# cvlab-stonybrook/s-volsdf

Hardware: AMD Instinct MI355X
Metric: rendered rays/sec (1024-ray batch, 128 samples) (higher is better)
Workload: dtype f32 (every product, forward and backward, as three fp16 MFMA products of two-piece fp16 operands with f32 accumulate; activation blocks hold both pieces: float32 accuracy class); 1 GPU; configs[1]: VolOpt.train_step (forward + MVS prior lookup + loss + backward + clip/guard/Adam), train mode, fast=1: 1024 rays/GPU x 128 coarse + 98 composited samples + 2048 eikonal points, 8x256 SDF MLP + 4x256 radiance MLP; mode=train, mlp_precision=fp16x2, launch=eager launches, rays_per_gpu=1024, rays_total=1024

## Files before the change

### include/svolsdf_hip.h

```cpp
#ifndef SVOLSDF_HIP_H
#define SVOLSDF_HIP_H

#include <stddef.h>
#include <stdint.h>

#ifdef __cplusplus
extern "C" {
#endif


#define SVS_EINVAL (-1)
#define SVS_ESHAPE (-2)
#define SVS_ENOCONV (-3)
#define SVS_EOVERFLOW (-4)

#define SVS_HOST

#define SVS_ABI_VERSION 101
int svs_version(void);
const char* svs_last_error_string(void);

int svs_set_deterministic(int on);
int svs_get_deterministic(void);

// ... 55 lines not shown
int svs_bg_points(const float* cam, int cam_stride, const float* dirs, int n_rays, int n_bg, const float* jitter,
                  float radius, float* z_bg, float* pts, float* depth_real, void* hip_stream);
int svs_bg_sdf_eval(const float* pts, int n_points, const float* stream, int precision, float* out0, float* feat_tiles,
                    float* hbuf, float* ghat7, float* pebuf, void* hip_stream);
size_t svs_bg_rbuf_bytes(int n_points);
int svs_bg_rgb_eval(int n_points, const float* view_dirs, int view_S, const float* feat_tiles, const float* stream,
                    int precision, float* rgb, float* rbuf, void* hip_stream);
int svs_bg_rgb_bwd(int n_points, const float* d_rgb, const float* rgb, const float* rbuf, const float* stream, int precision,
                   float* zbuf, float* feat_bar, float* absmax, void* hip_stream);
int svs_bg_sdf_bwd(int n_points, const float* d_out0, const float* feat_bar, const float* hbuf, const float* ghat7,
                   const float* stream, int precision, float* abuf, float* sbar_out, float* absmax, void* hip_stream);
int svs_composite_bg(int n_rays, int n_samples, int n_bg, const float* z, const float* z_max, const float* sdf,
                     const float* rgb, const float* normals, const float* depth_scale, const float* beta_param,
                     float beta_min, const float* z_bg, const float* bg_out0, const float* bg_rgb, const float* bg_depth,
                     float* weights, float* bg_trans, float* bg_weights, float* rgb_values, float* depth_values,
                     float* depth_values_all, float* depth_vals, float* normal_map, void* hip_stream);
int svs_composite_bg_bwd(int n_rays, int n_samples, int n_bg, const float* z, const float* z_max, const float* sdf,
                         const float* rgb, const float* depth_scale, const float* beta_param, float beta_min,
                         const float* z_bg, const float* bg_out0, const float* bg_rgb, const float* d_rgb_values,
                         const float* d_weights, const float* d_depth_values, const float* d_depth_all,
                         const float* bg_depth, float* d_sdf, float* d_rgb,
                         float* d_bg_out0, float* d_bg_rgb, float* d_beta_ray, float* d_beta_param, void* hip_stream);

typedef struct svs_wgrad_job {
  const float *a0, *b0; long long sa0, sb0;
  const float *a1, *b1; long long sa1, sb1;
  const float* b_extra; long long s_extra;
  int n_points, ldw;
  float *dW, *db;
  const float* absmax;
  const float *rec0, *rec1;
} svs_wgrad_job;
int svs_wgrad_multi(const svs_wgrad_job* jobs, int n_jobs, int precision, void* hip_stream);
int svs_wgrad(const float* a0, const float* b0, long long sa0, long long sb0, const float* a1, const float* b1,
              long long sa1, long long sb1, const float* b_extra, long long s_extra, int n_points, int precision,
              const float* absmax, const float* rec0, const float* rec1, float* dW, int ldw, float* db, void* hip_stream);

size_t svs_block_bytes(int n_points, int blocks_per_tile);
size_t svs_rgb_zbuf_bytes(int n_points);
size_t svs_sdf_ubuf_bytes(int n_points);
size_t svs_sdf_gbuf_bytes(int n_points);
int svs_rgb_bwd(int n_points, const float* d_rgb, const float* rgb, const float* rbuf, const float* stream, int precision,
                float* zbuf, float* feat_bar, float* d_normals, float* absmax, void* hip_stream);
int svs_sdf_bwd_a(const float* points, int n_points, const float* cam, int cam_stride, const float* dirs, const float* z,
                  int S, int n_rays, const float* d_grad, const unsigned char* clamp_mask, const float* hbuf,
                  const float* gbuf, const float* stream, int precision, float* ubuf, float* a2buf, float* pebuf,
                  float* absmax, void* hip_stream);
int svs_sdf_bwd_b(int n_points, const float* d_sdf, const unsigned char* clamp_mask, const float* feat_bar,
                  int n_feat_points, const float* hbuf, const float* gbuf, const float* a2buf, const float* ubuf,
                  const float* stream, int precision, float* abuf, float* sbar_out, float* absmax, void* hip_stream);
int svs_lin8_row0_grad(const float* hbuf, const float* ubuf, const float* sbar, int n_points, int precision, float* out257,
                       void* hip_stream);
int svs_unpack_wgrad(const float* dWk, const float* dbk, int ldw, int map, int rows, int cols, int row_off,
                     const float* weight_v, const float* weight_g, const float* row0, float* grad_v, float* grad_g,
                     float* grad_b, void* hip_stream);
typedef struct svs_unpack_job {
  const float *dWk, *dbk;
  int ldw, map, rows, cols, row_off;
  const float *weight_v, *weight_g, *row0;
  float *grad_v, *grad_g, *grad_b;
} svs_unpack_job;
int svs_unpack_wgrad_multi(const svs_unpack_job* jobs, int n_jobs, void* hip_stream);

size_t svs_adam_workspace_bytes(void);
int svs_clip_guard_adam(float* params, float* grads, float* exp_avg, float* exp_avg_sq, long long n, int step,
                        int* step_counter, double max_norm, double lr, double beta1, double beta2, double eps,
// ... 282 lines not shown
```

### s-volsdf_amd/csrc/svs_wgrad.hip

```cpp
#include "svs_common.h"
#include "svs_mlp_layout.h"
#include "svs_ticket.h"
#include "svs_wgrad_maps.h"
#include <cstdlib>
#include <type_traits>

namespace svs {
namespace wgrad {

struct Pair {
  const float* a;
  const float* b;
  size_t stride_a, stride_b;
};

struct Args {
  Pair p[2];
  int n_pairs;
  int n_tiles;
  int n_valid_points;
  const float* b_extra;
  size_t stride_extra;
  float* dW;
  int ldw;
// ... 138 lines not shown
  if constexpr (N > 0) {
    static_for<N - 1>(f);
    f(std::integral_constant<int, N - 1>{});
  }
}
__device__ __forceinline__ f16x8 frag_of(const Frag& v) { return __builtin_bit_cast(f16x8, v); }
__device__ __forceinline__ void lds_read128(f32x4& v, unsigned a) { asm volatile("ds_read_b128 %0, %1" : "=v"(v) : "v"(a)); }
__device__ __forceinline__ void lds_read32(float& v, unsigned a) { asm volatile("ds_read_b32 %0, %1" : "=v"(v) : "v"(a)); }
__device__ __forceinline__ void lds_wait() {
  asm volatile("s_waitcnt lgkmcnt(0)" ::: "memory");
  __builtin_amdgcn_sched_barrier(0);
}
__device__ __forceinline__ unsigned lds_addr(const void* p) {
  return (unsigned)(unsigned long long)SVS_LDS(const void, p);
}

__device__ __forceinline__ void scale_from_absmax(const float* absmax, float& s, float& inv_s) {
  s = 1.0f; inv_s = 1.0f;
  if (!absmax) return;
  int e = (int)((__float_as_uint(*absmax) >> 23) & 0xff);
  e = e < 16 ? 16 : (e > 250 ? 250 : e);
  s = __uint_as_float((unsigned)(268 - e) << 23);
  inv_s = __uint_as_float((unsigned)(e - 14) << 23);
}

struct Job {
  Pair p[2];
  const float* rec[2];
  int n_pairs;
  int n_tiles;
  int n_valid_points;
  int b_tiles;
  int col0;
  float* dW;
  int ldw;
  float* db;
  const float* absmax;
  int wg_begin, wg_count;
  det::Ticket ticket;
};
constexpr int kMaxJobs = 20;
struct MultiArgs { Job job[kMaxJobs]; int n_jobs; int touch; int reverse; };
static_assert(sizeof(MultiArgs) <= 4096, "kernel arguments");

constexpr int kThreadsW = 512;
constexpr int kRT = 2, kCT = 16;
static_assert(maps::plane_reads_ok(kPlane), "transposed reads of the operand planes: bank conflict");
static_assert(maps::narrow_reads_ok(kExtraPiece), "transposed reads of the narrow B image: bank conflict");
static_assert(kPlane % 256 == 0 && kNarrowImg % 256 == 0 && kExtraPiece % 256 == 0 && Ring<true>::kSlotAll % 256 == 0 &&
              Ring<false>::kSlotAll % 256 == 0, "every region the reads are offset by starts on a 256-byte bank row");

typedef const __attribute__((address_space(1))) void* gvoid;

template <bool GP>
__global__ __launch_bounds__(kThreadsW, 1) void wgrad_h2_multi_kernel(MultiArgs ma) {
  typedef Ring<GP> R;
  constexpr int kSlot = R::kSlot, kSlotAll = R::kSlotAll, kRing = R::kRing, kAhead = R::kAhead, kB = R::kB;
  extern __shared__ __attribute__((aligned(16))) unsigned char smem_h2[];
  int jj = 0;
  for (int q = 1; q < ma.n_jobs; ++q) if ((int)blockIdx.x >= ma.job[q].wg_begin) jj = q;
  const Job& a = ma.job[jj];
  const int wg = (int)blockIdx.x - a.wg_begin, nwg = a.wg_count;
  const int tid = threadIdx.x, lane = tid & 63;
  const int wave = __builtin_amdgcn_readfirstlane(tid >> 6);
  const bool narrow = a.b_tiles == 1;
  float s_grad, inv_s;
  scale_from_absmax(a.absmax, s_grad, inv_s);

  f32x4 acc[kRT][kCT];
#pragma unroll
  for (int o = 0; o < kRT; ++o)
#pragma unroll
    for (int i = 0; i < kCT; ++i) acc[o][i] = (f32x4)(0.0f);
  float bsum[kRT];
#pragma unroll
  for (int o = 0; o < kRT; ++o) bsum[o] = 0.0f;

  unsigned char* ring = smem_h2;

  const int rg = lane >> 4;
  const int rd_even = maps::plane_base(0, lane), rd_odd = maps::plane_base(1, lane);
  const int a_off = 1024 * kRT * wave;
  const int rx = maps::narrow_base(lane);
  const int wp = lane & 31, whf = lane >> 5;
  const int wxoff = maps::narrow_at(8 * (wave & 3) + 4 * whf, wp);
  const int n_ct = narrow ? 2 : kCT;

  const bool two_pairs = a.n_pairs == 2;
  const int my_tiles = a.n_tiles > wg ? (a.n_tiles - 1 - wg) / nwg + 1 : 0;
  const int n_items = two_pairs ? 2 * my_tiles : my_tiles;
  const int n_valid = a.n_valid_points;
  const bool has_db = a.db != nullptr;
  const bool rev = ma.reverse != 0;
  const float* const pa0 = a.p[0].a; const float* const pb0 = a.p[0].b;
  const float* const pa1 = a.p[1].a; const float* const pb1 = a.p[1].b;
  const size_t sa0 = a.p[0].stride_a, sb0 = a.p[0].stride_b, sa1 = a.p[1].stride_a, sb1 = a.p[1].stride_b;
  const float* const rec0 = a.rec[0]; const float* const rec1 = a.rec[1];
  const bool has_scale = a.absmax != nullptr;
  auto tile_of = [&](int item) {
    const int k = two_pairs ? item >> 1 : item;
    return rev ? wg + (my_tiles - 1 - k) * nwg : wg + k * nwg;
  };

  auto issue = [&](int item) {
    const int t = tile_of(item), pi = two_pairs ? item & 1 : 0;
    const float* pa = (pi ? pa1 : pa0) + (size_t)t * (pi ? sa1 : sa0);
    const float* pb = (pi ? pb1 : pb0) + (size_t)t * (pi ? sb1 : sb0);
    unsigned char* slot = ring + (item % kRing) * kSlotAll;
#pragma unroll
    for (int j = 0; j < 2 * R::kPlanes; ++j) {
      const int piece = wave + 8 * j;
      __builtin_amdgcn_global_load_lds((gvoid)(reinterpret_cast<const f32x4*>(pa) + piece * 64 + lane),
                                       SVS_LDS(void, slot + piece * 1024), 16, 0, 0);
      if (!narrow)
        __builtin_amdgcn_global_load_lds((gvoid)(reinterpret_cast<const f32x4*>(pb) + piece * 64 + lane),
                                         SVS_LDS(void, slot + kB + piece * 1024), 16, 0, 0);
    }
    if (narrow)
      __builtin_amdgcn_global_load_lds((gvoid)(reinterpret_cast<const f32x4*>(pb) + (wave & 3) * 64 + lane),
                                       SVS_LDS(void, slot + kB + (wave & 3) * 1024), 16, 0, 0);
    if (has_scale)
      __builtin_amdgcn_global_load_lds((gvoid)((pi ? rec1 : rec0) + (size_t)t * 64 + lane),
                                       SVS_LDS(void, slot + kSlot + wave * 256), 4, 0, 0);
  };
  unsigned sink = 0;
  auto touch = [&](int item) {
    const int t = tile_of(item), pi = two_pairs ? item & 1 : 0;
    const Pair& p = a.p[pi];
    constexpr int kLines = R::kPlanes * (kPlane / 128);
    const int nb = narrow ? 32 : kLines;
    const float* q = tid < kLines ? p.a + (size_t)t * p.stride_a + tid * 32
                                  : p.b + (size_t)t * p.stride_b + (tid - kLines) * 32;
    if (tid < kLines + nb) asm volatile("global_load_dword %0, %1, off" : "+v"(sink) : "v"(q) : "memory");
  };
  const int ops = (narrow ? 2 * R::kPlanes + 1 : 4 * R::kPlanes) + (has_scale ? 1 : 0);

  auto stage_factors = [&](int item) {
    unsigned char* slot = ring + (item % kRing) * kSlotAll;
    const int t = tile_of(item);
    const int live = n_valid - t * 32;
    float f = 1.0f;
    if (has_scale) {
      float rec;
      lds_read32(rec, lds_addr(slot + kSlot + wave * 256 + 4 * wp));
      lds_wait();
      const unsigned eb = (__float_as_uint(rec) >> 23) & 0xff;
      if (eb >= 20 && eb <= 240) f = __builtin_fminf(s_grad * __uint_as_float((254u << 23) - __float_as_uint(rec)), 32768.0f);
// ... 57 lines not shown
    const unsigned ftab = la + kSlot + kRecBytes + wave * 64;
    const unsigned a_even = la + a_off + rd_even, a_odd = la + a_off + rd_odd;
    const unsigned b_even = lb + rd_even, b_odd = lb + rd_odd;
    const unsigned n_rd = lb + kNarrowImg + rx;
    const bool want_bias = has_db && p0;
    const bool two = narrow;
    Frag fa[kRT], fam[kRT];
    f32x4 fraw;
    static_for<kRT>([&](auto oc) {
      constexpr int o = decltype(oc)::value;
      tr_issue<1024 * o>(fa[o], o & 1 ? a_odd : a_even);
      if (GP) tr_issue<kPlane + 1024 * o>(fam[o], o & 1 ? a_odd : a_even);
    });
    lds_read128(fraw, ftab + 16 * rg);
    issue_next();
    lds_wait();
    f16x8 ah[kRT], am[kRT];
#pragma unroll
    for (int o = 0; o < kRT; ++o) {
      ah[o] = frag_of(fa[o]) * __builtin_bit_cast(f16x8, fraw);
      am[o] = GP ? frag_of(fam[o]) * __builtin_bit_cast(f16x8, fraw) : ah[o];
      if (want_bias) {
#pragma unroll
        for (int j = 0; j < 4; ++j) {
          const f16x2 h2v = {ah[o][2 * j], ah[o][2 * j + 1]};
          bsum[o] = __builtin_amdgcn_fdot2(h2v, one2, bsum[o], false);
          if (GP) {
            const f16x2 m2v = {am[o][2 * j], am[o][2 * j + 1]};
            bsum[o] = __builtin_amdgcn_fdot2(m2v, one2, bsum[o], false);
          }
        }
      }
    }
    static_for<kCT>([&](auto ic) {
      constexpr int i = decltype(ic)::value;
      if (i < n_ct) {
        Frag fh, fm;
        if (!narrow) {
          tr_issue<1024 * i>(fh, i & 1 ? b_odd : b_even);
          if (GP) tr_issue<kPlane + 1024 * i>(fm, i & 1 ? b_odd : b_even);
        } else if constexpr (i < 2) {
          tr_issue<1024 * i>(fh, n_rd);
          tr_issue<kExtraPiece + 1024 * i>(fm, n_rd);
        }
        lds_wait();
        const f16x8 bh = frag_of(fh), bm = frag_of(fm);
        if (two || GP) {
#pragma unroll
          for (int o = 0; o < kRT; ++o) acc[o][i] = __builtin_amdgcn_mfma_f32_16x16x32_f16(ah[o], bm, acc[o][i], 0, 0, 0);
        }
        if (GP) {
#pragma unroll
          for (int o = 0; o < kRT; ++o) acc[o][i] = __builtin_amdgcn_mfma_f32_16x16x32_f16(am[o], bh, acc[o][i], 0, 0, 0);
        }
#pragma unroll
        for (int o = 0; o < kRT; ++o) acc[o][i] = __builtin_amdgcn_mfma_f32_16x16x32_f16(ah[o], bh, acc[o][i], 0, 0, 0);
      }
    });
  }
  asm volatile("s_waitcnt vmcnt(0)" :: "v"(sink) : "memory");
  const int fcol = lane & 15;
  det::wait_turn(a.ticket, wg);
  static_for<kCT>([&](auto ic) {
    constexpr int i = decltype(ic)::value;
    const int c = a.col0 + 16 * i + fcol;
    if (i < n_ct && c < a.ldw) {
#pragma unroll
      for (int o = 0; o < kRT; ++o)
#pragma unroll
        for (int r = 0; r < 4; ++r)
          atomicAdd(&a.dW[(size_t)(16 * (kRT * wave + o) + 4 * rg + r) * a.ldw + c], acc[o][i][r] * inv_s);
    }
  });
  if (a.db) {
#pragma unroll
    for (int o = 0; o < kRT; ++o) {
      float sum = bsum[o];
      sum += __shfl_xor(sum, 16);
      sum += __shfl_xor(sum, 32);
      if (lane < 16) atomicAdd(&a.db[16 * (kRT * wave + o) + lane], sum * inv_s);
    }
  }
  det::pass_turn(a.ticket, wg);
}

}

}
}

using namespace svs;
using namespace svs::wgrad;
namespace h2 = svs::wgrad::h2;

extern "C" {

int svs_wgrad_multi(const svs_wgrad_job* jobs, int n_jobs, int precision, void* hip_stream) {
  if (!jobs || n_jobs < 1) { set_error("svs_wgrad_multi: no jobs"); return SVS_EINVAL; }
  int n_expanded = 0;
  for (int j = 0; j < n_jobs; ++j) n_expanded += jobs[j].b_extra ? 2 : 1;
  if (n_expanded > h2::kMaxJobs) { set_error("svs_wgrad_multi: at most %d jobs (b_extra counts twice)", h2::kMaxJobs); return SVS_EINVAL; }
  for (int j = 0; j < n_jobs; ++j) {
    const svs_wgrad_job& q = jobs[j];
    if (!q.a0 || !q.b0 || !q.dW || q.n_points <= 0 || q.ldw < 256 || q.ldw > 288 || (q.b_extra && q.ldw < 288) || (q.a1 && !q.b1)) {
      set_error("svs_wgrad_multi: bad argument in job %d", j); return SVS_EINVAL;
    }
    if (mlp::is_h2(precision) && q.absmax && (!q.rec0 || (q.a1 && !q.rec1))) {
      set_error("svs_wgrad_multi: job %d has absmax but no scale records", j); return SVS_EINVAL;
    }
  }
  hipStream_t s = (hipStream_t)hip_stream;
  if (mlp::is_h2(precision)) {
    const bool gp = precision == mlp::kFmtF16x2;
    h2::MultiArgs ma;
    int n = 0;
    long long work[h2::kMaxJobs], total = 0;
    for (int j = 0; j < n_jobs; ++j) {
      const svs_wgrad_job& q = jobs[j];
      h2::Job& J = ma.job[n];
      J.p[0] = Pair{q.a0, q.b0, (size_t)q.sa0, (size_t)q.sb0};
      J.rec[0] = q.rec0; J.rec[1] = q.rec1;
      J.n_pairs = 1;
      if (q.a1) { J.p[1] = Pair{q.a1, q.b1, (size_t)q.sa1, (size_t)q.sb1}; J.n_pairs = 2; }
      else { J.p[1] = J.p[0]; J.rec[1] = J.rec[0]; }
      J.n_tiles = (q.n_points + 31) / 32; J.n_valid_points = q.n_points;
      J.b_tiles = 8; J.col0 = 0; J.dW = q.dW; J.ldw = q.ldw; J.db = q.db; J.absmax = q.absmax;
      work[n] = (long long)J.n_tiles * J.n_pairs * 10;
      total += work[n++];
      if (q.b_extra) {
        h2::Job& X = ma.job[n];
        X = J;
        X.p[0].b = q.b_extra; X.p[0].stride_b = (size_t)q.s_extra; X.n_pairs = 1;
        X.b_tiles = 1; X.col0 = 256; X.db = nullptr;
        work[n] = (long long)X.n_tiles * 6;
        total += work[n++];
      }
    }
    ma.n_jobs = n;
    static const int touch_env = [] { const char* e = getenv("SVS_WGRAD_TOUCH"); return e ? atoi(e) : 0; }();
    ma.touch = touch_env;
    static const int reverse_env = [] { const char* e = getenv("SVS_WGRAD_REVERSE"); return e ? atoi(e) : 0; }();
    ma.reverse = reverse_env;
    (void)total;
    const int n_wg_total = 256;
    int count[h2::kMaxJobs];
    int used = 0;
    for (int j = 0; j < n; ++j) { count[j] = 1; ++used; }
    while (used < n_wg_total) {
      int best = -1;
      double load = 0.0;
      for (int j = 0; j < n; ++j) {
        if (count[j] >= ma.job[j].n_tiles) continue;
        const double l = (double)work[j] / count[j];
        if (l > load) { load = l; best = j; }
      }
      if (best < 0) break;
      ++count[best]; ++used;
    }
    int begin = 0;
    for (int j = 0; j < n; ++j) {
      ma.job[j].wg_begin = begin; ma.job[j].wg_count = count[j];
      begin += count[j];
      ma.job[j].ticket = det::Ticket{nullptr, 0u, 0u};
    }
    if (deterministic()) {
      int owner[h2::kMaxJobs], n_owner = 0;
      for (int j = 0; j < n; ++j) {
// ... 20 lines not shown
    return check_launch("svs_wgrad_multi");
  }
  if (precision != mlp::kFmtF32) { set_error("svs_wgrad_multi: unknown precision %d", precision); return SVS_EINVAL; }
  for (int j = 0; j < n_jobs; ++j) {
    const svs_wgrad_job& q = jobs[j];
    Args a;
    a.p[0] = Pair{q.a0, q.b0, (size_t)q.sa0, (size_t)q.sb0};
    a.n_pairs = 1;
    if (q.a1) { a.p[1] = Pair{q.a1, q.b1, (size_t)q.sa1, (size_t)q.sb1}; a.n_pairs = 2; }
    a.n_tiles = (q.n_points + 31) / 32;
    a.n_valid_points = q.n_points;
    a.b_extra = q.b_extra; a.stride_extra = (size_t)q.s_extra;
    a.dW = q.dW; a.ldw = q.ldw; a.db = q.db;
    const int grid = a.n_tiles < 256 ? a.n_tiles : 256;
    a.ticket = det::Ticket{det::take_slots(1), 0u, (unsigned)grid};
    if (q.b_extra) {
      constexpr int lds = 2 * 32 * (260 + 292) * 4;
      static hipError_t e9 = hipFuncSetAttribute(reinterpret_cast<const void*>(wgrad_kernel<9>),
                                                 hipFuncAttributeMaxDynamicSharedMemorySize, lds);
      if (e9 != hipSuccess) { set_error("svs_wgrad_multi: hipFuncSetAttribute: %s", hipGetErrorString(e9)); return (int)e9; }
      wgrad_kernel<9><<<grid, 256, lds, s>>>(a);
    } else {
      constexpr int lds = 2 * 32 * (260 + 260) * 4;
      static hipError_t e8 = hipFuncSetAttribute(reinterpret_cast<const void*>(wgrad_kernel<8>),
                                                 hipFuncAttributeMaxDynamicSharedMemorySize, lds);
      if (e8 != hipSuccess) { set_error("svs_wgrad_multi: hipFuncSetAttribute: %s", hipGetErrorString(e8)); return (int)e8; }
      wgrad_kernel<8><<<grid, 256, lds, s>>>(a);
    }
    if (int rc = check_launch("svs_wgrad_multi")) return rc;
  }
  return SVS_OK;
}

int svs_wgrad(const float* a0, const float* b0, long long sa0, long long sb0, const float* a1, const float* b1,
              long long sa1, long long sb1, const float* b_extra, long long s_extra, int n_points, int precision,
              const float* absmax, const float* rec0, const float* rec1, float* dW, int ldw, float* db, void* hip_stream) {
  svs_wgrad_job q{a0, b0, sa0, sb0, a1, b1, sa1, sb1, b_extra, s_extra, n_points, ldw, dW, db, absmax, rec0, rec1};
  return svs_wgrad_multi(&q, 1, precision, hip_stream);
}

}
```

### s-volsdf_amd/svs_hip/lib.py

```python
import ctypes
import os
import re
from ctypes import POINTER, c_char_p, c_double, c_float, c_int, c_longlong, c_size_t, c_void_p

_HERE = os.path.dirname(os.path.abspath(__file__))
LIB_PATH = os.environ.get("SVS_LIB_PATH") or os.path.join(os.path.dirname(_HERE), "lib", "libsvolsdf_hip.so")
HEADER_PATH = os.path.join(os.path.dirname(os.path.dirname(_HERE)), "include", "svolsdf_hip.h")

_lib = None


class SvsError(RuntimeError):
    pass


_SCALARS = {"int": c_int, "float": c_float, "double": c_double, "size_t": c_size_t, "long long": c_longlong}
_POINTEES = set(_SCALARS) | {"void", "char", "unsigned char", "uint8_t", "short", "unsigned int", "unsigned long long"}
_TOKENS = re.compile(r"\w+|\*").findall
_NOT_A_DECLARATOR = re.compile(r"[^\w\s*]").search


def _ctype(base, stars, host, pointees):
    if stars == 0 and not host:
        return _SCALARS.get(base)
# ... 55 lines not shown
                raise SvsError(f"{HEADER_PATH}: enum: cannot parse `{item}`")
            constants[e.group(1)] = int(e.group(2))
        return " "
    text = re.sub(r"\benum\s*\{([^}]*)\}\s*;", enum, text)

    def struct(m):
        if m.group(1) != m.group(3):
            raise SvsError(f"{HEADER_PATH}: typedef struct {m.group(1)} is named {m.group(3)}")
        structs[m.group(1)] = _struct_fields(m.group(1), m.group(2))
        return " "
    text = re.sub(r"\btypedef\s+struct\s+(\w+)\s*\{([^}]*)\}\s*(\w+)\s*;", struct, text)

    pointees = _POINTEES | set(structs)
    for decl in filter(None, (d.strip() for d in text.split(";"))):
        m = re.fullmatch(r"([\w\s*]+?)\b(\w+)\s*\(([^()]*)\)", decl)
        if not m:
            raise SvsError(f"{HEADER_PATH}: cannot parse declaration `{' '.join(decl.split())[:80]}`")
        name, params = m.group(2), m.group(3).strip()
        _, restype = _declarator(m.group(1) + " " + name, pointees, f"{name}, return type")
        args = [] if params == "void" else [_declarator(p, pointees, name)[1] for p in params.split(",")]
        signatures[name] = (restype, args)
    return constants, structs, signatures


def _structure(cls_name, fields, c_name):
    return type(cls_name, (ctypes.Structure,), {"_fields_": fields, "__doc__": f"{c_name} of include/svolsdf_hip.h"})


try:
    with open(HEADER_PATH) as _f:
        _CONSTANTS, _STRUCTS, SIGNATURES = parse_header(_f.read())
    WGradJob = _structure("WGradJob", _STRUCTS["svs_wgrad_job"], "svs_wgrad_job")
    UnpackJob = _structure("UnpackJob", _STRUCTS["svs_unpack_job"], "svs_unpack_job")
    ABI_VERSION = _CONSTANTS["SVS_ABI_VERSION"]
    EINVAL, ESHAPE, ENOCONV, EOVERFLOW = (_CONSTANTS["SVS_E" + n] for n in ("INVAL", "SHAPE", "NOCONV", "OVERFLOW"))
    MMA_F32, MMA_F16X2, MMA_F16X2_HALF = (_CONSTANTS["SVS_MMA_" + n] for n in ("F32", "F16X2", "F16X2_HALF"))
    PAINT_BEST, PAINT_ONE_SIDED = (_CONSTANTS["SVS_PAINT_" + n] for n in ("BEST", "ONE_SIDED"))
except (OSError, KeyError) as _e:
    raise SvsError(f"{HEADER_PATH}: the binding is derived from this header and cannot do without it: {_e!r}") from _e


def load():
    global _lib
    if _lib is not None:
        return _lib
    import torch
    if not os.path.exists(LIB_PATH):
        raise SvsError(f"{LIB_PATH} not found: run `python s-volsdf_amd/build.py` (there is no CPU fallback)")
    lib = ctypes.CDLL(LIB_PATH)
    for name, (res, args) in SIGNATURES.items():
        fn = getattr(lib, name)
        fn.restype = res
        fn.argtypes = args
    have = lib.svs_version()
    if have != ABI_VERSION:
        raise SvsError(f"{LIB_PATH} has ABI version {have}, the header this binding reads declares {ABI_VERSION}: "
                       "rebuild with `python s-volsdf_amd/build.py --force`")
    if os.environ.get("SVS_DETERMINISTIC") == "1":
        lib.svs_set_deterministic(1)
    _lib = lib
    return lib


def deterministic():
    return bool(load().svs_get_deterministic())

# ... 6 lines not shown
```

### s-volsdf_amd/svs_hip/profiling.py

```python
import torch

from . import lib as _lib


class LaunchTimer:

    def __init__(self, names):
        self.names = list(names)
        self.events = {n: [] for n in self.names}
        self._orig = {}
        self.meta = {n: [] for n in self.names}

    def __enter__(self):
        L = _lib.load()
        for n in self.names:
            fn = getattr(L, n)
            self._orig[n] = fn
            setattr(L, n, self._wrap(n, fn))
        return self

    def _wrap(self, name, fn):
        def call(*args):
            e0, e1 = torch.cuda.Event(enable_timing=True), torch.cuda.Event(enable_timing=True)
            e0.record()
            rc = fn(*args)
            e1.record()
            self.events[name].append((e0, e1))
            self.meta[name].append(args)
            return rc
        return call

    def __exit__(self, *exc):
        L = _lib.load()
        for n, fn in self._orig.items():
            setattr(L, n, fn)
        return False

    def times_ms(self, name):
        return [a.elapsed_time(b) for a, b in self.events[name]]
```

### s-volsdf_amd/svs_hip/train.py

```python
import ctypes
import os

import torch

from . import lib as _lib
from .ops import _f32, _ptr, _ptr_array, _stream, default_precision, is_h2, F16X2, F16X2_HALF

KBLOCK = 128 * 64
KREC = 64


def block_stride(n_points):
    return ((n_points + 127) // 128) * 4 * KBLOCK
LDW = 288


def n_tiles_padded(n_points):
    return ((n_points + 127) // 128) * 4


def record_off(n_points, n_blocks, block):
    T = n_tiles_padded(n_points)
    return n_blocks * T * KBLOCK + block * T * KREC


def _off(t, n_floats):
    return t.data_ptr() + 4 * n_floats


class TrainStreams:
    def __init__(self, device, precision=None):
        L = _lib.load()
        self.precision = default_precision() if precision is None else int(precision)
        self.sdf = torch.empty(L.svs_stream_bytes(2) // 4, device=device)
        self.rgb = torch.empty(L.svs_stream_bytes(4) // 4, device=device)
        self.ws = torch.empty(L.svs_pack_workspace_bytes() // 4, device=device)

    def pack(self, sdf_params, rgb_params):
        L = _lib.load()
        sv, sg, sb = [[_f32(t) for t in x] if x is not None else None for x in sdf_params]
        rv, rg, rb = [[_f32(t) for t in x] if x is not None else None for x in rgb_params]
        self._keep = (sv, sg, sb, rv, rg, rb)
        st = _stream()
        _lib.check(L.svs_pack_stream(2, self.precision, _ptr_array(sv), _ptr_array(sg) if sg else None, _ptr_array(sb), _ptr(self.ws),
                                     _ptr(self.sdf), st), "svs_pack_stream(sdf train)")
        _lib.check(L.svs_pack_stream(4, self.precision, _ptr_array(rv), _ptr_array(rg) if rg else None, _ptr_array(rb), _ptr(self.ws),
                                     _ptr(self.rgb), st), "svs_pack_stream(rgb bwd)")


class WGradAccum:

    def __init__(self, device, slots=14):
        n = [slots * 256 * LDW, slots * 256, 260, 4]
        self.flat = torch.zeros(sum(n), device=device)
        parts = torch.split(self.flat, n)
        self.dWk = parts[0].view(slots, 256, LDW)
        self.dbk = parts[1].view(slots, 256)
        self.row0 = parts[2][:257]
        self.absmax = parts[3]

    def zero(self):
        self.flat.zero_()

    def bases(self):
        return self.dWk.data_ptr(), self.dbk.data_ptr(), self.absmax.data_ptr()


class _JobCache(dict):

    def memo(self, key, build):
        hit = self.get(key)
        if hit is None:
            if len(self) >= 64:
                self.clear()
            hit = self[key] = build()
        return hit


def _job_array(jobs):
    arr = (_lib.WGradJob * len(jobs))(*[_lib.WGradJob(*j) for j in jobs])
    return ctypes.cast(arr, ctypes.c_void_p), len(jobs), arr


def _f(addr, n_floats):
    return addr + 4 * n_floats


def wgrad_job(acc, slot, n_pts, amax, scaled, a0, sa0, b0, sb0, a1=None, sa1=0, b1=None, sb1=0, extra=None, sx=0,
              rec0=None, rec1=None):
    dWk, dbk, absmax = acc
    return (a0, b0, sa0, sb0, a1, b1, sa1, sb1, extra, sx, n_pts, LDW, _f(dWk, slot * 256 * LDW), _f(dbk, slot * 256),
            _f(absmax, amax) if scaled else None, rec0 if scaled else None, rec1 if scaled else None)


def rgb_wgrad_table(n_main, h2, acc, zbuf, feat, rbuf):
    LSm = block_stride(n_main)
    zrec = lambda l: _f(zbuf, record_off(n_main, 5, l))
    jobs = [wgrad_job(acc, 9, n_main, 1, h2, zbuf, KBLOCK, feat, KBLOCK, extra=_f(rbuf, 4 * LSm), sx=1024, rec0=zrec(0))]
    for l in range(1, 5):
        jobs.append(wgrad_job(acc, 9 + l, n_main, 1, h2, _f(zbuf, l * LSm), KBLOCK, _f(rbuf, (l - 1) * LSm), KBLOCK,
                              rec0=zrec(l)))
    return jobs


def sdf_wgrad_table(n_total, n_main, h2, acc, abuf, ubuf, pebuf, hbuf, gbuf, feat_bar):
    LS = block_stride(n_total)
    arec = lambda l: _f(abuf, record_off(n_total, 8, l))
    second = lambda l: dict(a1=_f(gbuf, l * LS), sa1=KBLOCK, b1=_f(ubuf, l * LS), sb1=KBLOCK,
                            rec1=_f(ubuf, record_off(n_total, 9, l)))
    jobs = [wgrad_job(acc, 0, n_total, 0, h2, abuf, KBLOCK, pebuf, KBLOCK, rec0=arec(0), **second(0))]
    for l in range(1, 8):
        jobs.append(wgrad_job(acc, l, n_total, 0, h2, _f(abuf, l * LS), KBLOCK, _f(hbuf, (l - 1) * LS), KBLOCK, rec0=arec(l),
                              **second(l)))
    jobs.append(wgrad_job(acc, 8, n_main, 2, h2, feat_bar, KBLOCK, _f(hbuf, 7 * LS), KBLOCK,
                          rec0=_f(feat_bar, record_off(n_main, 1, 0))))
    return jobs


BGRBUF = KBLOCK + 1024


def bg_wgrad_table(P, acc, abuf, zbuf, feat_bar, hbuf, pebuf, rbuf, feat):
    LS, Z2, T = block_stride(P), 2 * KBLOCK, n_tiles_padded(P)
    job = lambda slot, amax, *a, **k: wgrad_job(acc, slot, P, amax, True, *a, **k)
    arec = lambda l: _f(abuf, record_off(P, 8, l))
    jobs = [job(0, 0, abuf, KBLOCK, pebuf, KBLOCK, rec0=arec(0))]
    for l in range(1, 8):
        jobs.append(job(l, 0, _f(abuf, l * LS), KBLOCK, _f(hbuf, (l - 1) * LS), KBLOCK, rec0=arec(l)))
    jobs.append(job(8, 2, feat_bar, KBLOCK, _f(hbuf, 7 * LS), KBLOCK, rec0=_f(feat_bar, record_off(P, 1, 0))))
    zrec = lambda b: _f(zbuf, 2 * T * KBLOCK + b * T * KREC)
    jobs.append(job(9, 1, zbuf, Z2, feat, KBLOCK, rec0=zrec(0), extra=_f(rbuf, KBLOCK), sx=BGRBUF))
    jobs.append(job(10, 1, _f(zbuf, KBLOCK), Z2, rbuf, BGRBUF, rec0=zrec(1)))
    return jobs


def unpack_table(dWk, dbk, row0, layers, maps):
    jobs = []
    for net, l, slot, rows, cols, v, g, gv, gg, gb in layers:
        mp = maps[0] if (net == 0 and l == 4) else (maps[1] if (net == 1 and l == 0) else 0)
        last = net == 0 and l == 8
        jobs.append((_f(dWk, slot * 256 * LDW), _f(dbk, slot * 256), LDW, mp, rows, cols, 1 if last else 0, v, g,
                     row0 if last else None, gv, gg, gb))
    return jobs


def _unpack(accum, nets, maps, out, which=(0, 1)):
    dev = accum.dWk.device
    res, layers, keep = [], [], []
    for gi, (v, g, base) in enumerate(nets):
# ... 45 lines not shown
        self.ubuf = z(L.svs_sdf_ubuf_bytes(n_total))
        self.a2buf = z(L.svs_block_bytes(n_total, 8)) if not is_h2(self.streams.precision) else None
        self.abuf = z(L.svs_block_bytes(n_total, 8))
        self.pebuf = z(L.svs_block_bytes(n_total, 1))
        self.sbar = z(L.svs_block_bytes(n_total, 1) // (128 * 2))
        self.d_sdf_full = torch.zeros(n_total, device=self.dev)
        self.d_grad_full = torch.zeros(n_total, 3, device=self.dev)
        self._n = (n_total, n_main)

    def sdf_grad_out(self, n_total, n_main):
        self._alloc(n_total, n_main)
        return self.d_sdf_full[:n_main].view(n_main, 1)

    def grad_extra_out(self, n_total, n_main):
        self._alloc(n_total, n_main)
        return self.d_grad_full[n_main:]

    def accumulate(self, keep, d_rgb, d_sdf, d_grad_extra, wait=True, side=True, defer_wgrad=False, extra=None):
        L = _lib.load()
        src = keep["src"]
        n_total, n_main = src.n, keep["rgb"].shape[0]
        if n_main % 32:
            raise NotImplementedError("rays*samples of a group must be a multiple of 32")
        self._alloc(n_total, n_main)
        dev, acc, S = self.dev, self.accum, self.streams
        hbuf, gbuf, mask = keep["hbuf"], keep["gbuf"], keep["clamp_mask"]
        rbuf, feat = keep["rbuf"], keep["feat_tiles"]

        prec = S.precision
        h2 = is_h2(prec)

        cache, bases = self._job_cache, acc.bases()

        def wgrad_multi(key, build, more):
            own = cache.memo(key, build)
            arr, n, _ = cache.memo(("arr",) + key + ((more["key"],) if more else ()),
                                   lambda: _job_array(own + (more["jobs"] if more else [])))
            _lib.check(L.svs_wgrad_multi(arr, n, prec, _stream()), "svs_wgrad_multi")

        d_rgb = _f32(d_rgb)
        d_grad = self.d_grad_full
        d_normals = d_grad[:n_main]
        n_extra = 0 if d_grad_extra is None else d_grad_extra.shape[0]
        if n_main + n_extra != n_total:
            raise ValueError("d_grad_extra must cover the points that follow the ray samples")
        if n_extra and d_grad_extra.data_ptr() != d_grad[n_main:].data_ptr():
            torch.mul(_f32(d_grad_extra), 1.0, out=d_grad[n_main:])
        _lib.check(L.svs_rgb_bwd(n_main, _ptr(d_rgb), _ptr(keep["rgb"]), _ptr(rbuf), _ptr(S.rgb), prec, _ptr(self.zbuf),
                                 _ptr(self.feat_bar), _ptr(d_normals), _ptr(acc.absmax) if h2 else None, _stream()),
                   "svs_rgb_bwd")
        if d_sdf is not None and d_sdf.data_ptr() == self.d_sdf_full.data_ptr() and d_sdf.numel() == n_main:
            d_sdf_full = self.d_sdf_full
        else:
            d_sdf_full = torch.zeros(n_total, device=dev)
            if d_sdf is not None:
                d_sdf_full[:n_main] = _f32(d_sdf).reshape(-1)
        main = torch.cuda.current_stream()
        if self._side is None:
            self._side = torch.cuda.Stream(device=dev)
        if os.environ.get("SVS_RGB_WGRAD_SIDE", "1") == "0":
            side = False
        side_stream = self._side if side else main
        rkey = ("rgb", n_main, prec, self.zbuf.data_ptr(), feat.data_ptr(), rbuf.data_ptr(), bases[0])
        rgb_jobs = lambda: rgb_wgrad_table(n_main, h2, bases, _ptr(self.zbuf), _ptr(feat), _ptr(rbuf))
        deferred = None
        if defer_wgrad:
            ev_rgb = torch.cuda.Event(); ev_rgb.record(main)
            deferred = dict(rgb=dict(jobs=cache.memo(rkey, rgb_jobs), key=rkey), ev_rgb=ev_rgb)
            join = None
        else:
            fork = torch.cuda.Event(); fork.record(main)
            with torch.cuda.stream(side_stream):
                if side:
                    side_stream.wait_event(fork)
                if extra is not None:
                    side_stream.wait_event(extra["ev_rgb"])
                wgrad_multi(rkey, rgb_jobs, extra["rgb"] if extra else None)
                join = torch.cuda.Event(); join.record(side_stream)
        st = _stream()
        _lib.check(L.svs_sdf_bwd_a(*src.args(), _ptr(d_grad), _ptr(mask), _ptr(hbuf), _ptr(gbuf), _ptr(S.sdf), prec,
                                   _ptr(self.ubuf), _ptr(self.a2buf), _ptr(self.pebuf),
                                   _ptr(acc.absmax) if h2 else None, st), "svs_sdf_bwd_a")
        _lib.check(L.svs_sdf_bwd_b(n_total, _ptr(d_sdf_full), _ptr(mask), _ptr(self.feat_bar), n_main, _ptr(hbuf),
                                   _ptr(gbuf), _ptr(self.a2buf), _ptr(self.ubuf), _ptr(S.sdf), prec, _ptr(self.abuf),
                                   _ptr(self.sbar), _ptr(acc.absmax) if h2 else None, st),
                   "svs_sdf_bwd_b")
        _lib.check(L.svs_lin8_row0_grad(_ptr(hbuf), _ptr(self.ubuf), _ptr(self.sbar), n_total, prec, _ptr(acc.row0),
                                        _stream()), "svs_lin8_row0_grad")
        ev = self.timer_events = ([torch.cuda.Event(enable_timing=True) for _ in range(2)] if self.time_wgrad else None)
        if ev:
            ev[0].record()
        skey = ("sdf", n_total, n_main, prec, self.abuf.data_ptr(), self.ubuf.data_ptr(), self.pebuf.data_ptr(),
                hbuf.data_ptr(), gbuf.data_ptr(), self.feat_bar.data_ptr(), bases[0])
        sdf_jobs = lambda: sdf_wgrad_table(n_total, n_main, h2, bases, _ptr(self.abuf), _ptr(self.ubuf), _ptr(self.pebuf),
                                           _ptr(hbuf), _ptr(gbuf), _ptr(self.feat_bar))
        if defer_wgrad:
            deferred["sdf"] = dict(jobs=cache.memo(skey, sdf_jobs), key=skey)
            deferred["ev_all"] = torch.cuda.Event(); deferred["ev_all"].record(main)
            deferred["hold"] = self._hold = (d_grad, d_sdf_full, d_normals, d_rgb)
            return deferred
        if extra is not None:
            main.wait_event(extra["ev_all"])
        wgrad_multi(skey, sdf_jobs, extra["sdf"] if extra else None)
        if ev:
            ev[1].record()
        if wait and side:
            main.wait_event(join)
        self._hold = (d_grad, d_sdf_full, d_normals, d_rgb)
        return join

    def run(self, sdf_params, rgb_params, keep, d_rgb, d_sdf, d_grad_extra, out=None):
        self.streams.pack(sdf_params, rgb_params)
        self.accum.zero()
        self.accumulate(keep, d_rgb, d_sdf, d_grad_extra)
        return finalize(self.accum, sdf_params, rgb_params, out)


class BgBackward:
    def __init__(self, device, precision=None):
        L = _lib.load()
        self.dev = device
        self.precision = default_precision() if precision is None else int(precision)
        self.sdf_stream = torch.empty(L.svs_stream_bytes(6) // 4, device=device)
        self.rgb_stream = torch.empty(L.svs_stream_bytes(8) // 4, device=device)
        self.ws = torch.empty(L.svs_pack_workspace_bytes() // 4, device=device)
        self.accum = WGradAccum(device, slots=11)
        self.dWk, self.dbk, self.row0, self.absmax = self.accum.dWk, self.accum.dbk, self.accum.row0, self.accum.absmax
        self._job_cache = _JobCache()
        self._scratch = {}

    def pack(self, sdf_wb, rgb_wb):
        L = _lib.load()
        self._keep = []
        for which, (w, b), stream in ((6, sdf_wb, self.sdf_stream), (8, rgb_wb, self.rgb_stream)):
            w, b = [_f32(t) for t in w], [_f32(t) for t in b]
            self._keep += [w, b]
            _lib.check(L.svs_pack_stream(which, self.precision, _ptr_array(w), None, _ptr_array(b), _ptr(self.ws), _ptr(stream),
                                         _stream()), "svs_pack_stream(bg backward)")

    def zero(self):
        self.accum.zero()

    def _alloc(self, n, slot):
        cur = self._scratch.get(slot)
        if cur is not None and cur[0] == n:
            return cur[1:]
        L = _lib.load()
        z = lambda nbytes: torch.zeros(nbytes // 4, device=self.dev)
        cur = (n, z(L.svs_block_bytes(n, 2)),
               z(L.svs_block_bytes(n, 1)), z(L.svs_block_bytes(n, 8)), z(L.svs_block_bytes(n, 1) // (128 * 2)))
        self._scratch[slot] = cur
        return cur[1:]

    def accumulate(self, keep, d_bg_rgb, d_bg_out0, slot=0):
        L = _lib.load()
        P = keep["bg_rgb"].shape[0]
        zbuf, feat_bar, abuf, sbar = self._alloc(P, slot)
        st = _stream()
        hbuf, ghat7, pebuf, rbuf, feat = keep["bg_hbuf"], keep["bg_ghat7"], keep["bg_pebuf"], keep["bg_rbuf"], keep["bg_feat"]
        d_bg_rgb, d_bg_out0 = _f32(d_bg_rgb), _f32(d_bg_out0)
        prec = self.precision
        _lib.check(L.svs_bg_rgb_bwd(P, _ptr(d_bg_rgb), _ptr(keep["bg_rgb"]), _ptr(rbuf), _ptr(self.rgb_stream), prec, _ptr(zbuf),
                                    _ptr(feat_bar), _ptr(self.absmax), st), "svs_bg_rgb_bwd")
        _lib.check(L.svs_bg_sdf_bwd(P, _ptr(d_bg_out0), _ptr(feat_bar), _ptr(hbuf), _ptr(ghat7), _ptr(self.sdf_stream), prec,
                                    _ptr(abuf), _ptr(sbar), _ptr(self.absmax), st), "svs_bg_sdf_bwd")
        _lib.check(L.svs_lin8_row0_grad(_ptr(hbuf), None, _ptr(sbar), P, prec, _ptr(self.row0), st), "svs_lin8_row0_grad")
        ptrs = tuple(_ptr(t) for t in (abuf, zbuf, feat_bar, hbuf, pebuf, rbuf, feat))
        bases = self.accum.bases()
        arr, n, _ = self._job_cache.memo(("bg", P, prec) + ptrs + bases[:1],
                                         lambda: _job_array(bg_wgrad_table(P, bases, *ptrs)))
        _lib.check(L.svs_wgrad_multi(arr, n, prec, st), "svs_wgrad_multi(bg)")
        self._hold = getattr(self, "_hold", {})
        self._hold[slot] = (d_bg_rgb, d_bg_out0)

    def finalize(self, sdf_wb, rgb_wb, out=None):
        if out is not None:
            out = [[(gw, None, gb) for gw, gb in group] for group in out]
        res = _unpack(self.accum, ((sdf_wb[0], None, 0), (rgb_wb[0], None, 9)), (3, 4), out)
        return tuple([(gw, gb) for gw, _, gb in group] for group in res)


def algorithmic_bytes_per_point(precision=None):
    precision = default_precision() if precision is None else precision
    if is_h2(precision):
        half = 512 if precision == F16X2_HALF else 1024
        pair = 1024
        return {"svs_sdf_bwd_a": 8 * half + 9 * half + pair,
                "svs_sdf_bwd_b": 8 * half + 8 * half + 8 * half + half + 8 * half,
                "wgrad_sdf": 8 * (half + half + half + half) + half + half,
                "wgrad_radiance": 5 * half + 4 * half + half + 128,
                "svs_lin8_row0_grad": pair + half,
                "svs_sdf_outputs": 8 * pair + 8 * pair + 8 * half + pair}
    blk = 1024
    return {"svs_sdf_bwd_a": (8 + 8 + 9 + 8 + 1) * blk, "svs_sdf_bwd_b": (8 + 8 + 1 + 1 + 8) * blk,
            "wgrad_sdf": (8 * 4 + 2) * blk, "wgrad_radiance": (5 + 4 + 1) * blk + 128, "svs_lin8_row0_grad": 2 * blk,
            "svs_sdf_outputs": (8 + 8 + 8 + 1) * blk}
```

Baseline: 303,400 rays/s.

## Skip dead row/column tiles in weight-gradient kernel using per-job extents

```diff
diff --git a/include/svolsdf_hip.h b/include/svolsdf_hip.h
--- a/include/svolsdf_hip.h
+++ b/include/svolsdf_hip.h
@@ -111,6 +111,9 @@
   const float *rec0, *rec1;
 } svs_wgrad_job;
 int svs_wgrad_multi(const svs_wgrad_job* jobs, int n_jobs, int precision, void* hip_stream);
+typedef struct svs_wgrad_extent { int rows, cols; } svs_wgrad_extent;
+int svs_wgrad_multi_extents(const svs_wgrad_job* jobs, int n_jobs, const svs_wgrad_extent* extents, int precision,
+                            void* hip_stream);
 int svs_wgrad(const float* a0, const float* b0, long long sa0, long long sb0, const float* a1, const float* b1,
               long long sa1, long long sb1, const float* b_extra, long long s_extra, int n_points, int precision,
               const float* absmax, const float* rec0, const float* rec1, float* dW, int ldw, float* db, void* hip_stream);
diff --git a/s-volsdf_amd/csrc/svs_wgrad.hip b/s-volsdf_amd/csrc/svs_wgrad.hip
--- a/s-volsdf_amd/csrc/svs_wgrad.hip
+++ b/s-volsdf_amd/csrc/svs_wgrad.hip
@@ -194,6 +194,7 @@
   int n_valid_points;
   int b_tiles;
   int col0;
+  int a_live, b_live;
   float* dW;
   int ldw;
   float* db;
@@ -204,6 +205,14 @@
 constexpr int kMaxJobs = 20;
 struct MultiArgs { Job job[kMaxJobs]; int n_jobs; int touch; int reverse; };
 static_assert(sizeof(MultiArgs) <= 4096, "kernel arguments");
+
+constexpr int kWidePrice = 1000, kNarrowPrice = 600, kPriceFloor = 0, kLonePrice = 700;
+inline int item_price(int a_live, int b_live, bool gp) {
+  const int copy = gp ? kWidePrice * (a_live + b_live) / 32 : kWidePrice;
+  const int mfma = (a_live > 8 ? kWidePrice : kLonePrice) * (b_live <= 4 ? b_live : 16) / 16;
+  const int frac = copy > mfma ? copy : mfma;
+  return kPriceFloor + (kWidePrice - kPriceFloor) * frac / kWidePrice;
+}
 
 constexpr int kThreadsW = 512;
 constexpr int kRT = 2, kCT = 16;
@@ -246,7 +255,19 @@
   const int rx = maps::narrow_base(lane);
   const int wp = lane & 31, whf = lane >> 5;
   const int wxoff = maps::narrow_at(8 * (wave & 3) + 4 * whf, wp);
-  const int n_ct = narrow ? 2 : kCT;
+  enum : int { kCopyA0 = 1, kCopyA1 = 2, kCopyB0 = 4, kCopyB1 = 8, kFewBit = 16 };
+  constexpr int kFew = 4;
+  int cfg_of;
+  {
+    const int a_live = a.a_live, b_live = a.b_live;
+    const int n_ct = kRT * wave >= a_live ? 0 : narrow ? 2 : b_live;
+    cfg_of = (!GP || wave < a_live ? kCopyA0 : 0) | (!GP || wave + 8 < a_live ? kCopyA1 : 0) |
+             (!narrow && (!GP || wave < b_live) ? kCopyB0 : 0) | (!narrow && (!GP || wave + 8 < b_live) ? kCopyB1 : 0) |
+             (!narrow && n_ct <= kFew ? kFewBit : 0) | (n_ct << 8);
+  }
+  int cfg = __builtin_amdgcn_readfirstlane(cfg_of);
+  auto cfg_in_loop = [&]() { asm volatile("" : "+s"(cfg)); return cfg; };
+  const int n_all = narrow ? 2 : kCT;
 
   const bool two_pairs = a.n_pairs == 2;
   const int my_tiles = a.n_tiles > wg ? (a.n_tiles - 1 - wg) / nwg + 1 : 0;
@@ -269,12 +290,14 @@
     const float* pa = (pi ? pa1 : pa0) + (size_t)t * (pi ? sa1 : sa0);
     const float* pb = (pi ? pb1 : pb0) + (size_t)t * (pi ? sb1 : sb0);
     unsigned char* slot = ring + (item % kRing) * kSlotAll;
+    const int c = cfg_in_loop();
 #pragma unroll
     for (int j = 0; j < 2 * R::kPlanes; ++j) {
       const int piece = wave + 8 * j;
-      __builtin_amdgcn_global_load_lds((gvoid)(reinterpret_cast<const f32x4*>(pa) + piece * 64 + lane),
-                                       SVS_LDS(void, slot + piece * 1024), 16, 0, 0);
-      if (!narrow)
+      if (c & (j & 1 ? kCopyA1 : kCopyA0))
+        __builtin_amdgcn_global_load_lds((gvoid)(reinterpret_cast<const f32x4*>(pa) + piece * 64 + lane),
+                                         SVS_LDS(void, slot + piece * 1024), 16, 0, 0);
+      if (c & (j & 1 ? kCopyB1 : kCopyB0))
         __builtin_amdgcn_global_load_lds((gvoid)(reinterpret_cast<const f32x4*>(pb) + piece * 64 + lane),
                                          SVS_LDS(void, slot + kB + piece * 1024), 16, 0, 0);
     }
@@ -398,9 +421,31 @@
         }
       }
     }
+    if (const int c = cfg_in_loop(); c & kFewBit) {
+      const int n_few = c >> 8;
+      static_for<kFew>([&](auto ic) {
+        constexpr int i = decltype(ic)::value;
+        if (i < n_few) {
+          Frag fh, fm;
+          tr_issue<1024 * i>(fh, i & 1 ? b_odd : b_even);
+          if (GP) tr_issue<kPlane + 1024 * i>(fm, i & 1 ? b_odd : b_even);
+          lds_wait();
+          const f16x8 bh = frag_of(fh), bm = frag_of(fm);
+          if (GP) {
+#pragma unroll
+            for (int o = 0; o < kRT; ++o) acc[o][i] = __builtin_amdgcn_mfma_f32_16x16x32_f16(ah[o], bm, acc[o][i], 0, 0, 0);
+#pragma unroll
+            for (int o = 0; o < kRT; ++o) acc[o][i] = __builtin_amdgcn_mfma_f32_16x16x32_f16(am[o], bh, acc[o][i], 0, 0, 0);
+          }
+#pragma unroll
+          for (int o = 0; o < kRT; ++o) acc[o][i] = __builtin_amdgcn_mfma_f32_16x16x32_f16(ah[o], bh, acc[o][i], 0, 0, 0);
+        }
+      });
+      continue;
+    }
     static_for<kCT>([&](auto ic) {
       constexpr int i = decltype(ic)::value;
-      if (i < n_ct) {
+      if (i < n_all) {
         Frag fh, fm;
         if (!narrow) {
           tr_issue<1024 * i>(fh, i & 1 ? b_odd : b_even);
@@ -426,6 +471,7 @@
   }
   asm volatile("s_waitcnt vmcnt(0)" :: "v"(sink) : "memory");
   const int fcol = lane & 15;
+  const int n_ct = cfg >> 8, a_live = a.a_live;
   det::wait_turn(a.ticket, wg);
   static_for<kCT>([&](auto ic) {
     constexpr int i = decltype(ic)::value;
@@ -433,9 +479,11 @@
     if (i < n_ct && c < a.ldw) {
 #pragma unroll
       for (int o = 0; o < kRT; ++o)
-#pragma unroll
-        for (int r = 0; r < 4; ++r)
-          atomicAdd(&a.dW[(size_t)(16 * (kRT * wave + o) + 4 * rg + r) * a.ldw + c], acc[o][i][r] * inv_s);
+        if (kRT * wave + o < a_live) {
+#pragma unroll
+          for (int r = 0; r < 4; ++r)
+            atomicAdd(&a.dW[(size_t)(16 * (kRT * wave + o) + 4 * rg + r) * a.ldw + c], acc[o][i][r] * inv_s);
+        }
     }
   });
   if (a.db) {
@@ -444,7 +492,7 @@
       float sum = bsum[o];
       sum += __shfl_xor(sum, 16);
       sum += __shfl_xor(sum, 32);
-      if (lane < 16) atomicAdd(&a.db[16 * (kRT * wave + o) + lane], sum * inv_s);
+      if (lane < 16 && kRT * wave + o < a_live) atomicAdd(&a.db[16 * (kRT * wave + o) + lane], sum * inv_s);
     }
   }
   det::pass_turn(a.ticket, wg);
@@ -461,8 +509,14 @@
 
 extern "C" {
 
-int svs_wgrad_multi(const svs_wgrad_job* jobs, int n_jobs, int precision, void* hip_stream) {
+int svs_wgrad_multi_extents(const svs_wgrad_job* jobs, int n_jobs, const svs_wgrad_extent* extents, int precision,
+                            void* hip_stream) {
   if (!jobs || n_jobs < 1) { set_error("svs_wgrad_multi: no jobs"); return SVS_EINVAL; }
+  for (int j = 0; extents && j < n_jobs; ++j)
+    if (extents[j].rows < 1 || extents[j].rows > 256 || extents[j].cols < 1 || extents[j].cols > 256) {
+      set_error("svs_wgrad_multi: extent %d x %d of job %d is not within 1..256", extents[j].rows, extents[j].cols, j);
+      return SVS_EINVAL;
+    }
   int n_expanded = 0;
   for (int j = 0; j < n_jobs; ++j) n_expanded += jobs[j].b_extra ? 2 : 1;
   if (n_expanded > h2::kMaxJobs) { set_error("svs_wgrad_multi: at most %d jobs (b_extra counts twice)", h2::kMaxJobs); return SVS_EINVAL; }
@@ -491,14 +545,16 @@
       else { J.p[1] = J.p[0]; J.rec[1] = J.rec[0]; }
       J.n_tiles = (q.n_points + 31) / 32; J.n_valid_points = q.n_points;
       J.b_tiles = 8; J.col0 = 0; J.dW = q.dW; J.ldw = q.ldw; J.db = q.db; J.absmax = q.absmax;
-      work[n] = (long long)J.n_tiles * J.n_pairs * 10;
+      J.a_live = extents ? (extents[j].rows + 15) / 16 : 16;
+      J.b_live = extents ? (extents[j].cols + 15) / 16 : 16;
+      work[n] = (long long)J.n_tiles * J.n_pairs * h2::item_price(J.a_live, J.b_live, gp);
       total += work[n++];
       if (q.b_extra) {
         h2::Job& X = ma.job[n];
         X = J;
         X.p[0].b = q.b_extra; X.p[0].stride_b = (size_t)q.s_extra; X.n_pairs = 1;
         X.b_tiles = 1; X.col0 = 256; X.db = nullptr;
-        work[n] = (long long)X.n_tiles * 6;
+        work[n] = (long long)X.n_tiles * h2::kNarrowPrice;
         total += work[n++];
       }
     }
@@ -585,6 +641,10 @@
   return SVS_OK;
 }
 
+int svs_wgrad_multi(const svs_wgrad_job* jobs, int n_jobs, int precision, void* hip_stream) {
+  return svs_wgrad_multi_extents(jobs, n_jobs, nullptr, precision, hip_stream);
+}
+
 int svs_wgrad(const float* a0, const float* b0, long long sa0, long long sb0, const float* a1, const float* b1,
               long long sa1, long long sb1, const float* b_extra, long long s_extra, int n_points, int precision,
               const float* absmax, const float* rec0, const float* rec1, float* dW, int ldw, float* db, void* hip_stream) {
diff --git a/s-volsdf_amd/svs_hip/lib.py b/s-volsdf_amd/svs_hip/lib.py
--- a/s-volsdf_amd/svs_hip/lib.py
+++ b/s-volsdf_amd/svs_hip/lib.py
@@ -111,6 +111,7 @@
         _CONSTANTS, _STRUCTS, SIGNATURES = parse_header(_f.read())
     WGradJob = _structure("WGradJob", _STRUCTS["svs_wgrad_job"], "svs_wgrad_job")
     UnpackJob = _structure("UnpackJob", _STRUCTS["svs_unpack_job"], "svs_unpack_job")
+    WGradExtent = _structure("WGradExtent", _STRUCTS["svs_wgrad_extent"], "svs_wgrad_extent")
     ABI_VERSION = _CONSTANTS["SVS_ABI_VERSION"]
     EINVAL, ESHAPE, ENOCONV, EOVERFLOW = (_CONSTANTS["SVS_E" + n] for n in ("INVAL", "SHAPE", "NOCONV", "OVERFLOW"))
     MMA_F32, MMA_F16X2, MMA_F16X2_HALF = (_CONSTANTS["SVS_MMA_" + n] for n in ("F32", "F16X2", "F16X2_HALF"))
diff --git a/s-volsdf_amd/svs_hip/profiling.py b/s-volsdf_amd/svs_hip/profiling.py
--- a/s-volsdf_amd/svs_hip/profiling.py
+++ b/s-volsdf_amd/svs_hip/profiling.py
@@ -11,22 +11,25 @@
         self._orig = {}
         self.meta = {n: [] for n in self.names}
 
+    ALIASES = {"svs_wgrad_multi": (("svs_wgrad_multi_extents", lambda a: a[:2] + a[3:]),)}
+
     def __enter__(self):
         L = _lib.load()
         for n in self.names:
-            fn = getattr(L, n)
-            self._orig[n] = fn
-            setattr(L, n, self._wrap(n, fn))
+            for entry, meta in ((n, None),) + self.ALIASES.get(n, ()):
+                fn = getattr(L, entry)
+                self._orig[entry] = fn
+                setattr(L, entry, self._wrap(n, fn, meta))
         return self
 
-    def _wrap(self, name, fn):
+    def _wrap(self, name, fn, meta=None):
         def call(*args):
             e0, e1 = torch.cuda.Event(enable_timing=True), torch.cuda.Event(enable_timing=True)
             e0.record()
             rc = fn(*args)
             e1.record()
             self.events[name].append((e0, e1))
-            self.meta[name].append(args)
+            self.meta[name].append(meta(args) if meta else args)
             return rc
         return call
 
diff --git a/s-volsdf_amd/svs_hip/train.py b/s-volsdf_amd/svs_hip/train.py
--- a/s-volsdf_amd/svs_hip/train.py
+++ b/s-volsdf_amd/svs_hip/train.py
@@ -35,12 +35,14 @@
         self.sdf = torch.empty(L.svs_stream_bytes(2) // 4, device=device)
         self.rgb = torch.empty(L.svs_stream_bytes(4) // 4, device=device)
         self.ws = torch.empty(L.svs_pack_workspace_bytes() // 4, device=device)
+        self.shapes = None
 
     def pack(self, sdf_params, rgb_params):
         L = _lib.load()
         sv, sg, sb = [[_f32(t) for t in x] if x is not None else None for x in sdf_params]
         rv, rg, rb = [[_f32(t) for t in x] if x is not None else None for x in rgb_params]
         self._keep = (sv, sg, sb, rv, rg, rb)
+        self.shapes = ([tuple(t.shape) for t in sv], [tuple(t.shape) for t in rv])
         st = _stream()
         _lib.check(L.svs_pack_stream(2, self.precision, _ptr_array(sv), _ptr_array(sg) if sg else None, _ptr_array(sb), _ptr(self.ws),
                                      _ptr(self.sdf), st), "svs_pack_stream(sdf train)")
@@ -77,9 +79,14 @@
         return hit
 
 
-def _job_array(jobs):
+def _job_array(jobs, extents=None):
     arr = (_lib.WGradJob * len(jobs))(*[_lib.WGradJob(*j) for j in jobs])
-    return ctypes.cast(arr, ctypes.c_void_p), len(jobs), arr
+    if extents is None:
+        return ctypes.cast(arr, ctypes.c_void_p), len(jobs), arr, None
+    if len(extents) != len(jobs):
+        raise ValueError("one output extent per weight-gradient job")
+    ext = (_lib.WGradExtent * len(jobs))(*[_lib.WGradExtent(*e) for e in extents])
+    return ctypes.cast(arr, ctypes.c_void_p), len(jobs), (arr, ext), ctypes.cast(ext, ctypes.c_void_p)
 
 
 def _f(addr, n_floats):
@@ -115,6 +122,14 @@
     jobs.append(wgrad_job(acc, 8, n_main, 2, h2, feat_bar, KBLOCK, _f(hbuf, 7 * LS), KBLOCK,
                           rec0=_f(feat_bar, record_off(n_main, 1, 0))))
     return jobs
+
+
+def sdf_wgrad_extents(shapes):
+    return [(r, c) for r, c in shapes[:8]] + [(shapes[8][0] - 1, shapes[8][1])]
+
+
+def rgb_wgrad_extents(shapes):
+    return [(r, min(c, 256)) for r, c in shapes]
 
 
 BGRBUF = KBLOCK + 1024
@@ -226,11 +241,15 @@
 
         cache, bases = self._job_cache, acc.bases()
 
-        def wgrad_multi(key, build, more):
+        def wgrad_multi(key, build, more, extents):
             own = cache.memo(key, build)
-            arr, n, _ = cache.memo(("arr",) + key + ((more["key"],) if more else ()),
-                                   lambda: _job_array(own + (more["jobs"] if more else [])))
-            _lib.check(L.svs_wgrad_multi(arr, n, prec, _stream()), "svs_wgrad_multi")
+            ext = tuple(extents) * (2 if more else 1) if extents is not None else None
+            arr, n, _, earr = cache.memo(("arr", ext) + key + ((more["key"],) if more else ()),
+                                         lambda: _job_array(own + (more["jobs"] if more else []), ext))
+            _lib.check(L.svs_wgrad_multi_extents(arr, n, earr, prec, _stream()), "svs_wgrad_multi")
+
+        sdf_ext = sdf_wgrad_extents(S.shapes[0]) if S.shapes else None
+        rgb_ext = rgb_wgrad_extents(S.shapes[1]) if S.shapes else None
 
         d_rgb = _f32(d_rgb)
         d_grad = self.d_grad_full
@@ -269,7 +288,7 @@
                     side_stream.wait_event(fork)
                 if extra is not None:
                     side_stream.wait_event(extra["ev_rgb"])
-                wgrad_multi(rkey, rgb_jobs, extra["rgb"] if extra else None)
+                wgrad_multi(rkey, rgb_jobs, extra["rgb"] if extra else None, rgb_ext)
                 join = torch.cuda.Event(); join.record(side_stream)
         st = _stream()
         _lib.check(L.svs_sdf_bwd_a(*src.args(), _ptr(d_grad), _ptr(mask), _ptr(hbuf), _ptr(gbuf), _ptr(S.sdf), prec,
@@ -295,7 +314,7 @@
             return deferred
         if extra is not None:
             main.wait_event(extra["ev_all"])
-        wgrad_multi(skey, sdf_jobs, extra["sdf"] if extra else None)
+        wgrad_multi(skey, sdf_jobs, extra["sdf"] if extra else None, sdf_ext)
         if ev:
             ev[1].record()
         if wait and side:
@@ -361,9 +380,9 @@
         _lib.check(L.svs_lin8_row0_grad(_ptr(hbuf), None, _ptr(sbar), P, prec, _ptr(self.row0), st), "svs_lin8_row0_grad")
         ptrs = tuple(_ptr(t) for t in (abuf, zbuf, feat_bar, hbuf, pebuf, rbuf, feat))
         bases = self.accum.bases()
-        arr, n, _ = self._job_cache.memo(("bg", P, prec) + ptrs + bases[:1],
-                                         lambda: _job_array(bg_wgrad_table(P, bases, *ptrs)))
-        _lib.check(L.svs_wgrad_multi(arr, n, prec, st), "svs_wgrad_multi(bg)")
+        arr, n, _, _ = self._job_cache.memo(("bg", P, prec) + ptrs + bases[:1],
+                                            lambda: _job_array(bg_wgrad_table(P, bases, *ptrs)))
+        _lib.check(L.svs_wgrad_multi_extents(arr, n, None, prec, st), "svs_wgrad_multi(bg)")
         self._hold = getattr(self, "_hold", {})
         self._hold[slot] = (d_bg_rgb, d_bg_out0)
 
```

New measurement: 305,400 rays/s, median of 6. No clear change (+0.7%).
